# pynbody/topsy

Hardware: AMD Instinct MI355X
Metric: particles/sec splatted to 1024^2 buffer (higher is better)
Workload: dtype f32

## Files before the change

### include/topsy_splat.h

```cpp
#ifndef TOPSY_SPLAT_H
#define TOPSY_SPLAT_H

#include <stdint.h>

#ifdef __cplusplus
extern "C" {
#endif

typedef struct tsp_context tsp_context;

enum {
    TSP_OK = 0,
    TSP_EINVAL = -1,
    TSP_EHIP = -2,
    TSP_ENODEV = -3,
    TSP_ESTATE = -4,
    TSP_ECOMM = -5,
    TSP_ENOMEM = -6
};

enum {
    TSP_MODE_WEIGHTED = 0,
    TSP_MODE_DEPTH = 1,
    TSP_MODE_RGB = 2
// ... 120 lines not shown
int tsp_content_sort(tsp_context *ctx, int kind, float scale, int64_t *n_finite, int64_t *n_nonpositive);
int tsp_content_values(tsp_context *ctx, const int64_t *ranks, int n_ranks, float *out);

typedef struct {
    int64_t n_particles;
    int64_t n_small;
    int64_t n_mid;
    int64_t n_huge;
    int64_t n_culled;
    int64_t n_fragments;
    double ms_stream, ms_mid, ms_huge, ms_total;
    double ms_mega;
    int64_t n_mega;
    int64_t n_fragments_stream, n_fragments_mid, n_fragments_huge, n_fragments_mega;
    int64_t n_chunk_culled;
} tsp_stats;
int tsp_get_stats(tsp_context *ctx, tsp_stats *out);
int tsp_set_option(tsp_context *ctx, const char *name, int64_t value);

int tsp_measure_read_bandwidth(tsp_context *ctx, int64_t bytes, int iters, double *gbps_out);

#define TSP_UNIQUE_ID_BYTES 128
int tsp_comm_unique_id(char *id_out);
int tsp_comm_init(tsp_context *ctx, int n_ranks, int rank, const char *id);
int tsp_comm_reduce_image(tsp_context *ctx, int root, double *gpu_ms_out);
int tsp_comm_destroy(tsp_context *ctx);
int tsp_set_reduced_image(tsp_context *ctx, const float *sum);

typedef struct tsp_group tsp_group;
int tsp_group_create(int n_devices, const int *device_ids, int resolution, int n_channels, tsp_group **out);
// ... 26 lines not shown
```

### topsy_amd/_native.py

```python
import ctypes
import os

import numpy as np

_HERE = os.path.dirname(os.path.abspath(__file__))
LIB_PATH = os.environ.get("TOPSY_SPLAT_LIB") or os.path.join(_HERE, "libtopsy_splat.so")

MODE_WEIGHTED, MODE_DEPTH, MODE_RGB = 0, 1, 2
PIPE_DEFAULT, PIPE_GENERIC = 0, 1
SAMPLE_BILINEAR_MIP0, SAMPLE_BILINEAR_MIP = 0x10, 0x20
UNIQUE_ID_BYTES = 128
ABI_VERSION = 109
PRESENT_SCALAR, PRESENT_BIVARIATE, PRESENT_RGB, PRESENT_RGB_HDR = 0, 1, 2, 3
LAYER_QUAD, LAYER_LINES = 0, 1


class SurfaceParams(ctypes.Structure):
    _fields_ = [("smoothing_scale", ctypes.c_double), ("depth_scale", ctypes.c_float),
                ("light_direction", ctypes.c_float * 3), ("light_color", ctypes.c_float * 3), ("ambient_color", ctypes.c_float * 3),
                ("vmin", ctypes.c_float), ("vmax", ctypes.c_float), ("weighted_average", ctypes.c_int), ("log_scale", ctypes.c_int),
                ("lut_rgba", ctypes.POINTER(ctypes.c_float)), ("n_lut", ctypes.c_int)]


class PresentBase(ctypes.Structure):
    _fields_ = [("map", ctypes.c_int), ("vmin", ctypes.c_float), ("vmax", ctypes.c_float), ("density_vmin", ctypes.c_float),
                ("density_vmax", ctypes.c_float), ("gamma", ctypes.c_float), ("log_scale", ctypes.c_int), ("weighted", ctypes.c_int),
                ("lut_rgba", ctypes.POINTER(ctypes.c_float)), ("n_lut", ctypes.c_int)]
# ... 10 lines not shown

class BackendUnavailable(RuntimeError):
    """libtopsy_splat.so could not be loaded, or no MI355X-class GPU is visible."""


class BackendError(RuntimeError):
    """A C-ABI call returned a negative status."""


class Stats(ctypes.Structure):
    _fields_ = [("n_particles", ctypes.c_int64), ("n_small", ctypes.c_int64), ("n_mid", ctypes.c_int64),
                ("n_huge", ctypes.c_int64), ("n_culled", ctypes.c_int64), ("n_fragments", ctypes.c_int64),
                ("ms_stream", ctypes.c_double), ("ms_mid", ctypes.c_double), ("ms_huge", ctypes.c_double),
                ("ms_total", ctypes.c_double), ("ms_mega", ctypes.c_double), ("n_mega", ctypes.c_int64),
                ("n_fragments_stream", ctypes.c_int64), ("n_fragments_mid", ctypes.c_int64),
                ("n_fragments_huge", ctypes.c_int64), ("n_fragments_mega", ctypes.c_int64), ("n_chunk_culled", ctypes.c_int64)]

    def as_dict(self):
        return {k: getattr(self, k) for k, _ in self._fields_}


_fp = ctypes.POINTER(ctypes.c_float)
_i64p = ctypes.POINTER(ctypes.c_int64)
_u8p = ctypes.POINTER(ctypes.c_uint8)
_ctx = ctypes.c_void_p

SIGNATURES = {
    "tsp_last_error": (ctypes.c_char_p, []),
    "tsp_version": (ctypes.c_int, []),
    "tsp_stats_size": (ctypes.c_int, []),
    "tsp_device_count": (ctypes.c_int, []),
# ... 632 lines not shown
```

### topsy_amd/csrc/tsp_api.hip

```cpp
#include <stdarg.h>
#include <string.h>

#include <algorithm>
#include <cmath>
#include <vector>

#include "tsp_internal.h"

namespace tsp {

static thread_local char g_err[1024] = "";

void set_error(const char *fmt, ...) {
    va_list ap;
    va_start(ap, fmt);
    vsnprintf(g_err, sizeof(g_err), fmt, ap);
    va_end(ap);
}

int ensure_array(float **p, int64_t n) {
    if (*p) {
        TSP_HIP(hipFree(*p));
        *p = nullptr;
    }
// ... 123 lines not shown
    p.n = 0;
    ctx->ws.bounds_valid = false;
    ctx->surface_keys = false;
    ctx->strata_offsets.clear();
    ctx->cell_offsets.clear();
    ctx->cell_bits = 0;
}

}

using namespace tsp;

extern "C" {

const char *tsp_last_error(void) { return g_err; }
int tsp_version(void) { return 109; }
int tsp_stats_size(void) { return (int)sizeof(tsp_stats); }

int tsp_device_count(void) {
    int n = 0;
    if (hipGetDeviceCount(&n) != hipSuccess) {
        set_error("hipGetDeviceCount failed");
        return TSP_ENODEV;
    }
    return n;
}

static int create_resources(tsp_context *ctx, int device_id, int resolution, int n_channels) {
    hipDeviceProp_t prop;
    TSP_HIP(hipGetDeviceProperties(&prop, device_id));
    ctx->cu_count = prop.multiProcessorCount > 0 ? prop.multiProcessorCount : 256;
// ... 313 lines not shown

    Camera cam;
    for (int i = 0; i < 12; ++i) cam.m[i] = M[i];
    cam.sf = scale_factor;
    cam.R = ctx->R;
    cam.Rf = (float)ctx->R;
    cam.halfR = 0.5f * cam.Rf;

    TSP_HIP(hipEventRecord(ctx->ev[0], ctx->stream));
    if (clear)
        TSP_HIP(hipMemsetAsync(ctx->image64, 0, (size_t)ctx->R * ctx->R * ctx->C * sizeof(double), ctx->stream));
    TSP_HIP(hipMemsetAsync(ctx->counters, 0, sizeof(Counters), ctx->stream));
    ctx->stats = tsp_stats{};
    ctx->stats.n_particles = total;
    ctx->chunk_culled_particles = 0;
    int rc = TSP_OK;
    if (total > 0) {
        const int rule = (flags & TSP_SAMPLE_BILINEAR_MIP0) ? 1 : ((flags & TSP_SAMPLE_BILINEAR_MIP) ? 2 : 0);
        if ((flags & TSP_PIPE_GENERIC) || rule != 0) {
            std::vector<int64_t> pack(3 * (size_t)nr + 1);
            int64_t acc = 0;
            for (int i = 0; i < nr; ++i) {
                pack[i] = s[i];
                pack[nr + i] = l[i];
                pack[2 * nr + i] = acc;
                acc += l[i];
            }
            pack[3 * nr] = acc;
            if (ctx->ws.range_capacity < (int64_t)pack.size()) {
                const int64_t cap = (int64_t)pack.size() * 2 + 64;
// ... 11 lines not shown
    }
    if (rc) return rc;
    if ((rc = launch_image_convert(ctx, true))) return rc;
    ctx->image_is_reduced = false;
    TSP_HIP(hipEventRecord(ctx->ev[1], ctx->stream));
    TSP_HIP(hipStreamSynchronize(ctx->stream));
    float ms = 0.f;
    TSP_HIP(hipEventElapsedTime(&ms, ctx->ev[0], ctx->ev[1]));
    ctx->stats.ms_total = ms;
    Counters hc;
    TSP_HIP(hipMemcpy(&hc, ctx->counters, sizeof(hc), hipMemcpyDeviceToHost));
    ctx->stats.n_small = (int64_t)hc.n_small;
    ctx->stats.n_mid = (int64_t)hc.n_mid;
    ctx->stats.n_huge = (int64_t)hc.n_huge;
    ctx->stats.n_mega = 0;
    ctx->stats.n_culled = (int64_t)hc.n_culled + ctx->chunk_culled_particles;
    ctx->stats.n_chunk_culled = ctx->chunk_culled_particles;
    ctx->stats.n_fragments = (int64_t)hc.n_fragments;
    ctx->stats.n_fragments_stream = (int64_t)hc.n_frag_class[0];
    ctx->stats.n_fragments_mid = (int64_t)hc.n_frag_class[1];
    ctx->stats.n_fragments_huge = (int64_t)hc.n_frag_class[2];
    ctx->stats.n_fragments_mega = (int64_t)hc.n_frag_class[3];
    if (gpu_ms_out) *gpu_ms_out = ms;
    return TSP_OK;
}

int tsp_read_image(tsp_context *ctx, float *out) {
    TSP_REQUIRE(ctx && out, TSP_EINVAL, "NULL argument");
    TSP_HIP(hipSetDevice(ctx->device));
    TSP_HIP(hipMemcpy(out, ctx->image, (size_t)ctx->R * ctx->R * ctx->C * sizeof(float), hipMemcpyDeviceToHost));
    return TSP_OK;
}
// ... 361 lines not shown
    }
    if (!strcmp(name, "h2_walk")) {
        TSP_REQUIRE(value == 0 || value == 1, TSP_EINVAL, "%s out of range", name);
        ctx->h2_walk = (int)value;
        return TSP_OK;
    }
    if (!strcmp(name, "reorder_interleave")) {
        TSP_REQUIRE(value >= 0 && value <= 2, TSP_EINVAL, "%s out of range", name);
        ctx->reorder_interleave = (int)value;
        return TSP_OK;
    }
    if (!strcmp(name, "chunk_cull")) {
        ctx->chunk_cull = value != 0;
        return TSP_OK;
    }
    if (!strcmp(name, "overlap_mid_huge")) {
        ctx->overlap_mid_huge = value != 0;
        return TSP_OK;
    }
    if (!strcmp(name, "use_quantity")) {
        ctx->use_quantity = value != 0;
        return TSP_OK;
    }
    if (!strcmp(name, "active_channels")) {
        TSP_REQUIRE((value == 2 || value == 4) && value <= ctx->Ccap, TSP_EINVAL, "bad channel count %lld", (long long)value);
        ctx->C = (int)value;
        return TSP_OK;
    }
    set_error("unknown option '%s'", name);
    return TSP_EINVAL;
// ... 10 lines not shown
```

### topsy_amd/csrc/tsp_group.hip

```cpp
#include <algorithm>
#include <string>
#include <thread>
#include <vector>

#include "tsp_internal.h"

struct tsp_group {
    std::vector<tsp_context *> ctx;
    std::vector<int64_t> bounds;
    bool rccl = false;
    bool needs_reduce = false;
    int R = 0, Ccap = 0;
};

namespace {

using tsp::set_error;

template <typename F> int for_each_context(tsp_group *grp, F fn) {
    const int G = (int)grp->ctx.size();
    std::vector<int> rc(G, TSP_OK);
    std::vector<std::string> msg(G);
    std::vector<std::thread> th;
    th.reserve(G);
// ... 215 lines not shown
        return tsp_upload_band_magnitudes(grp->ctx[g], n_bands, cut.data(), weights);
    });
}

int tsp_group_get_stats(tsp_group *grp, tsp_stats *out) {
    TSP_REQUIRE(grp && out, TSP_EINVAL, "NULL argument");
    tsp_stats t = {};
    for (tsp_context *c : grp->ctx) {
        tsp_stats s;
        const int rc = tsp_get_stats(c, &s);
        if (rc) return rc;
        t.n_particles += s.n_particles; t.n_small += s.n_small; t.n_mid += s.n_mid; t.n_huge += s.n_huge; t.n_culled += s.n_culled;
        t.n_fragments += s.n_fragments; t.n_mega += s.n_mega;
        t.n_fragments_stream += s.n_fragments_stream; t.n_fragments_mid += s.n_fragments_mid;
        t.n_fragments_huge += s.n_fragments_huge; t.n_fragments_mega += s.n_fragments_mega; t.n_chunk_culled += s.n_chunk_culled;
        t.ms_stream = std::max(t.ms_stream, s.ms_stream); t.ms_mid = std::max(t.ms_mid, s.ms_mid);
        t.ms_huge = std::max(t.ms_huge, s.ms_huge); t.ms_mega = std::max(t.ms_mega, s.ms_mega);
        t.ms_total = std::max(t.ms_total, s.ms_total);
    }
    *out = t;
    return TSP_OK;
}

}
```

### topsy_amd/csrc/tsp_internal.h

```cpp
#pragma once
#include <hip/hip_runtime.h>
#include <stdint.h>

#include <initializer_list>
#include <vector>
#include <stdio.h>
#include <string>

#include "../../include/topsy_splat.h"
#include "tsp_math.h"

namespace tsp {

void set_error(const char *fmt, ...);

#define TSP_HIP(call)                                                                          \
    do {                                                                                       \
        hipError_t e_ = (call);                                                                \
        if (e_ != hipSuccess) {                                                                \
            tsp::set_error("%s failed: %s (%s:%d)", #call, hipGetErrorString(e_), __FILE__, __LINE__); \
            return TSP_EHIP;                                                                   \
        }                                                                                      \
    } while (0)

// ... 16 lines not shown
    bool wm_valid = false, wrgb_valid = false;
};

constexpr int BOUNDS_BLOCK = 512;

struct Record {
    float pcx, pcy, P, w0, w1;
};
struct Record4 {
    float pcx, pcy, P, w0, w1, w2;
};

struct Counters {
    unsigned long long n_small, n_mid, n_huge, n_culled, n_fragments, huge_count, next_chunk, mid_odd_weights;
    unsigned long long n_frag_class[4];
};

struct Workspace {
    void *mid_geom = nullptr, *mid_w = nullptr;
    int64_t mid_capacity = 0;
    void *huge_geom = nullptr, *huge_w = nullptr;
    int64_t huge_capacity = 0;
    void *hband_geom = nullptr, *hband_w = nullptr;
    int *hband_count = nullptr;
    int64_t hband_stride = 0; int hband_bands = 0;
    void *mband_geom = nullptr, *mband_w = nullptr;
    int *mband_count = nullptr;
    long long *mband_base = nullptr;
    int64_t mband_capacity = 0;
    int mtile_capacity = 0;
// ... 54 lines not shown
    bool count_fragments = false;
    float p_small = 16.0f;
    int64_t huge_band_budget = 6ll << 30;
    int huge_variant = 1;
    int h2_walk = 1;
    int huge_split = 0;
    int reorder_interleave = 2;
    int stream_blocks_per_cu = 0;
    int debug_gather_full_lut = 0;
    double mid_item_scale = 0.35;
    float mid_narrow_px = 64.0f;
    int mid_item_records = 0;
    int stream_batch_chunks = 8;
    bool chunk_cull = true;
    int64_t chunk_culled_particles = 0;
    bool overlap_mid_huge = false;
    int64_t slice_records = 0;
    int debug_fail_stage = 0;
    int64_t debug_fail_alloc = 0;
    int stream_occ[3][2] = {};
    bool debug_no_raster = false;
    int cu_count = 256;
    void *comm = nullptr;
    int n_ranks = 1, rank = 0;
    bool image_is_reduced = false;
};

namespace tsp {
struct DeviceScratch {
    void *p = nullptr;
// ... 62 lines not shown
```

### topsy_amd/csrc/tsp_pipeline.hip

```cpp
#include <string.h>

#include <algorithm>
#include <type_traits>
#include <vector>

#include "tsp_pipeline.h"

namespace tsp {

template <int CTRL, int ROW_MASK> __device__ __forceinline__ int dpp_or(int identity, int v) {
    return __builtin_amdgcn_update_dpp(identity, v, CTRL, ROW_MASK, 0xf, false);
}
template <typename Op> __device__ __forceinline__ int wave_scan_bits(int v, int identity, Op op) {
    v = op(v, dpp_or<0x111, 0xf>(identity, v));
    v = op(v, dpp_or<0x112, 0xf>(identity, v));
    v = op(v, dpp_or<0x114, 0xf>(identity, v));
    v = op(v, dpp_or<0x118, 0xf>(identity, v));
    v = op(v, dpp_or<0x142, 0xa>(identity, v));
    v = op(v, dpp_or<0x143, 0xc>(identity, v));
    return v;
}
__device__ __forceinline__ float wave_min(float v) {
    const int r = wave_scan_bits(__float_as_int(v), __float_as_int(__builtin_inff()),
                                 [](int a, int b) { return __float_as_int(fminf(__int_as_float(a), __int_as_float(b))); });
// ... 45 lines not shown
    int count_frag;
    int emit_small;
    const int *alive;
    const unsigned long long *cull_info;
};

static_assert(CHUNK == BOUNDS_BLOCK, "block bounds are kept per chunk-sized block");
constexpr int T23_FLOATS = 17 * 17 + 9 * 9;

struct CullArgs {
    const int64_t *ranges; int n_ranges; int n_chunks;
    Camera cam;
    const float4 *bounds; int64_t n_particles;
    int *alive; unsigned long long *info;
    int *wg_count;
};

__device__ __forceinline__ bool box_outside_view(const Camera &c, float4 lo, float4 hi) {
    if (!(c.sf > 0.0f)) return false;
    const float bx = 0.5f * lo.x + 0.5f * hi.x, by = 0.5f * lo.y + 0.5f * hi.y, bz = 0.5f * lo.z + 0.5f * hi.z;
    const float ex = 0.5f * hi.x - 0.5f * lo.x, ey = 0.5f * hi.y - 0.5f * lo.y, ez = 0.5f * hi.z - 0.5f * lo.z;
    const float s = (c.sf * lo.w) * 2.0f;
    const float px = 4.0f / c.Rf;
    bool out = false;
#pragma unroll
    for (int row = 0; row < 3; ++row) {
        const float a = c.m[4 * row] * bx, b = c.m[4 * row + 1] * by, d = c.m[4 * row + 2] * bz, t = c.m[4 * row + 3];
        const float centre = ((a + b) + d) + t;
        const float ext = (__builtin_fabsf(c.m[4 * row]) * ex + __builtin_fabsf(c.m[4 * row + 1]) * ey) + __builtin_fabsf(c.m[4 * row + 2]) * ez;
        const float mag = (((__builtin_fabsf(a) + __builtin_fabsf(b)) + __builtin_fabsf(d)) + __builtin_fabsf(t)) + ext;
        if (row < 2) {
            const float reach = (ext + s) + (1e-4f * (mag + s) + px);
            out = out || (centre - reach > 1.0f) || (centre + reach < -1.0f);
        } else {
            const float reach = ext + (1e-4f * mag + 1e-6f);
            out = out || (centre - reach > 1.0f) || (centre + reach < 0.0f);
        }
    }
    return out;
}

__device__ __forceinline__ bool chunk_alive(const CullArgs &a, int c, int &cnt) {
    const int n_ranges = a.n_ranges;
    const int64_t *starts = a.ranges, *lens = starts + n_ranges, *cprefix = starts + 2 * n_ranges;
    int lo = 0, hi = n_ranges - 1;
    while (lo < hi) {
        const int mid = (lo + hi + 1) >> 1;
        if (cprefix[mid] <= c) lo = mid; else hi = mid - 1;
    }
    const int64_t in_range = (int64_t)(c - cprefix[lo]) * CHUNK;
    const int64_t first = starts[lo] + in_range;
    cnt = (int)min((int64_t)CHUNK, lens[lo] - in_range);
    const int64_t b0 = first / BOUNDS_BLOCK, b1 = (first + cnt - 1) / BOUNDS_BLOCK;
    float4 blo = a.bounds[2 * b0], bhi = a.bounds[2 * b0 + 1];
    if (b1 != b0) {
        const float4 l1 = a.bounds[2 * b1], h1 = a.bounds[2 * b1 + 1];
        blo = make_float4(fminf(blo.x, l1.x), fminf(blo.y, l1.y), fminf(blo.z, l1.z), fmaxf(blo.w, l1.w));
        bhi = make_float4(fmaxf(bhi.x, h1.x), fmaxf(bhi.y, h1.y), fmaxf(bhi.z, h1.z), 0.0f);
    }
    return !box_outside_view(a.cam, blo, bhi);
}

template <int PASS>
__global__ __launch_bounds__(256) void chunk_cull_kernel(CullArgs a) {
    __shared__ int s_cnt[4];
    const int c = blockIdx.x * 256 + threadIdx.x, lane = threadIdx.x & 63, wv = threadIdx.x >> 6;
    int cnt = 0;
    const bool alive = (c < a.n_chunks) && chunk_alive(a, c, cnt);
    const unsigned long long m = __ballot(alive);
    if (lane == 0) s_cnt[wv] = __popcll(m);
    if (PASS == 0) {
        unsigned long long dropped = alive ? 0ull : (unsigned long long)cnt;
        for (int o = 32; o; o >>= 1) dropped += __shfl_xor((long long)dropped, o);
        if (lane == 0 && dropped) atomicAdd(&a.info[1], dropped);
    }
    __syncthreads();
    if (PASS == 0) {
        if (threadIdx.x == 0) a.wg_count[blockIdx.x] = s_cnt[0] + s_cnt[1] + s_cnt[2] + s_cnt[3];
    } else if (alive) {
        int pos = a.wg_count[blockIdx.x] + __popcll(m & ((1ull << lane) - 1ull));
        for (int w = 0; w < wv; ++w) pos += s_cnt[w];
        a.alive[pos] = c;
    }
}

__global__ __launch_bounds__(1024) void chunk_cull_scan_kernel(int *wg_count, int n, unsigned long long *info) {
    __shared__ int s_wave[16];
    __shared__ int s_carry;
    const int tid = threadIdx.x, lane = tid & 63, wv = tid >> 6;
    if (tid == 0) s_carry = 0;
    __syncthreads();
    for (int base = 0; base < n; base += 1024) {
        const int i = base + tid;
        const int v = i < n ? wg_count[i] : 0;
        int incl = v;
        for (int o = 1; o < 64; o <<= 1) {
            const int t = __shfl_up(incl, o);
            if (lane >= o) incl += t;
        }
        if (lane == 63) s_wave[wv] = incl;
        __syncthreads();
        int before = s_carry;
        for (int w = 0; w < wv; ++w) before += s_wave[w];
        if (i < n) wg_count[i] = before + incl - v;
        __syncthreads();
        if (tid == 1023) s_carry = before + incl;
        __syncthreads();
    }
    if (tid == 0) info[0] = (unsigned long long)s_carry;
}

template <int MODE, int WC>
__global__ __launch_bounds__(SBLOCK, TSP_S_OCC) void splat_stream_kernel(StreamArgs ) {
    typedef const __attribute__((address_space(4))) StreamArgs CArgs;
    auto KA = []() -> CArgs * {
        CArgs *p = (CArgs *)__builtin_amdgcn_kernarg_segment_ptr();
        asm volatile("" : "+s"(p));
        return p;
    };
    constexpr int C = (MODE == TSP_MODE_RGB) ? 4 : 2;
    constexpr int NW = (MODE == TSP_MODE_RGB) ? 2 : 1;
    constexpr int WIN = WinSize<WC>::value;
    extern __shared__ __attribute__((aligned(16))) double smem_d[];
    double *win = smem_d;
// ... 373 lines not shown
        n_small += __shfl_xor((long long)n_small, o);
        n_cull += __shfl_xor((long long)n_cull, o);
        n_frag += __shfl_xor((long long)n_frag, o);
    }
    if (lane == 0) {
        Counters *cntp = KA()->cnt;
        if (n_small) atomicAdd(&cntp->n_small, n_small);
        if (n_cull) atomicAdd(&cntp->n_culled, n_cull);
        if (n_frag) { atomicAdd(&cntp->n_fragments, n_frag); atomicAdd(&cntp->n_frag_class[0], n_frag); }
#ifdef TSP_S_DEBUG
        if (dbg_slots) atomicAdd(&cntp->n_frag_class[1], dbg_slots);
#endif
    }
}

__global__ __launch_bounds__(256) void rect_count_corners_kernel(const float4 *__restrict__ geom, long long n, int R, int *__restrict__ D) {
    const long long i = (long long)blockIdx.x * 256 + threadIdx.x;
    if (i >= n) return;
    const float4 g = geom[i];
    const float half = 0.5f * __builtin_fabsf(g.z);
    int ilo, ihi, jlo, jhi;
    cover_range(g.x, half, R, ilo, ihi);
    cover_range(g.y, half, R, jlo, jhi);
    if (ilo > ihi || jlo > jhi) return;
    const int S = R + 1;
    atomicAdd(&D[jlo * S + ilo], 1);
    atomicAdd(&D[jlo * S + ihi + 1], -1);
    atomicAdd(&D[(jhi + 1) * S + ilo], -1);
    atomicAdd(&D[(jhi + 1) * S + ihi + 1], 1);
}
// ... 76 lines not shown
        pack[2 * n_ranges + i] = n_chunks64;
        n_chunks64 += (h_lens[i] + CHUNK - 1) / CHUNK;
    }
    pack[3 * n_ranges] = n_chunks64;
    TSP_REQUIRE(n_chunks64 < (1ll << 30), TSP_EINVAL, "too many chunks");
    const int n_chunks = (int)n_chunks64;
    int rc;
    if ((rc = check_workspace(ctx))) return rc;
    if (ws.range_capacity < (int64_t)pack.size()) {
        const int64_t cap = (int64_t)pack.size() * 2 + 64;
        if ((rc = alloc_group(ctx, {{"range_prefix", (void **)&ws.range_prefix, (size_t)cap * sizeof(int64_t)}}, {{&ws.range_capacity, cap}}))) return rc;
    }
    TSP_HIP(hipMemcpyAsync(ws.range_prefix, pack.data(), pack.size() * sizeof(int64_t), hipMemcpyHostToDevice, st));
    if (ws.chunk_capacity < n_chunks) {
        const int64_t cap = (int64_t)n_chunks + n_chunks / 4 + 64;
        if ((rc = alloc_group(ctx, {{"alive_list", (void **)&ws.alive_list, (size_t)(cap + cap / 256 + 2) * sizeof(int)}}, {{&ws.chunk_capacity, cap}})))
            return rc;
    }
    if ((rc = ensure_weights(ctx, MODE == TSP_MODE_RGB))) return rc;
    if (ws.mid_capacity == 0 && (rc = alloc_list(ctx, &ws.mid_geom, &ws.mid_w, &ws.mid_capacity, std::max<int64_t>(total / 4, 1 << 16),
                                                 SITE("mid_geom"), SITE("mid_w"))))
        return rc;
    if (ws.huge_capacity == 0 && (rc = alloc_list(ctx, &ws.huge_geom, &ws.huge_w, &ws.huge_capacity, std::max<int64_t>(total / 16, 1 << 16),
                                                  SITE("huge_geom"), SITE("huge_w"))))
        return rc;

    Particles parts = ctx->p;
    if (!ctx->use_quantity) parts.q = nullptr;
    const bool second_channel = (MODE == TSP_MODE_DEPTH) || (MODE == TSP_MODE_RGB) || (ctx->p.q != nullptr && ctx->use_quantity);
    const int WCr = (MODE == TSP_MODE_RGB) ? 4 : (second_channel ? 2 : 1);
    const int WIN = (WCr == 1) ? WinSize<1>::value : WinSize<C>::value;
    const size_t smem_s = (size_t)WCr * WIN * WIN * sizeof(double) + T23_FLOATS * sizeof(float);
    if (!(ctx->kernel_attr_done & (1u << MODE))) {
        TSP_HIP(hipFuncSetAttribute((const void *)splat_stream_kernel<MODE, C>, hipFuncAttributeMaxDynamicSharedMemorySize, (int)((size_t)C * WinSize<C>::value * WinSize<C>::value * sizeof(double) + T23_FLOATS * sizeof(float))));
        TSP_HIP(hipFuncSetAttribute((const void *)splat_stream_kernel<MODE, 1>, hipFuncAttributeMaxDynamicSharedMemorySize, (int)((size_t)WinSize<1>::value * WinSize<1>::value * sizeof(double) + T23_FLOATS * sizeof(float))));
        ctx->kernel_attr_done |= 1u << MODE;
    }

    const bool cull = ctx->chunk_cull && n_chunks >= 4096;
    unsigned long long cull_info_h[2] = {0, 0};
    ctx->chunk_culled_particles = 0;
    TSP_HIP(hipEventRecord(ctx->ev[7], st));
    if (cull) {
        if ((rc = ensure_block_bounds(ctx))) return rc;
        if (!ws.cull_info && (rc = alloc_group(ctx, {{"cull_info", (void **)&ws.cull_info, 2 * sizeof(unsigned long long)}}, {}))) return rc;
        TSP_HIP(hipMemsetAsync(ws.cull_info, 0, 2 * sizeof(unsigned long long), st));
        CullArgs ca;
        ca.ranges = ws.range_prefix; ca.n_ranges = n_ranges; ca.n_chunks = n_chunks; ca.cam = cam;
        ca.bounds = ws.block_bounds; ca.n_particles = ctx->p.n; ca.alive = ws.alive_list; ca.info = ws.cull_info;
        ca.wg_count = ws.alive_list + ws.chunk_capacity;
        const int n_wg = (n_chunks + 255) / 256;
        hipLaunchKernelGGL(chunk_cull_kernel<0>, dim3(n_wg), dim3(256), 0, st, ca);
        hipLaunchKernelGGL(chunk_cull_scan_kernel, dim3(1), dim3(1024), 0, st, ca.wg_count, n_wg, ws.cull_info);
        hipLaunchKernelGGL(chunk_cull_kernel<1>, dim3(n_wg), dim3(256), 0, st, ca);
        TSP_HIP(hipGetLastError());
    }

    Counters hc, carry;
    memset(&carry, 0, sizeof(carry));
    for (int attempt = 0; attempt < 2; ++attempt) {
        StreamArgs sa;
        sa.p = parts;
        sa.alive = cull ? ws.alive_list : nullptr; sa.cull_info = ws.cull_info;
        sa.ranges = ws.range_prefix; sa.n_ranges = n_ranges; sa.n_chunks = n_chunks;
        const int min_cpb = std::max(1, std::min(8, n_chunks / (ctx->cu_count * 2)));
        int per_cu = ctx->stream_blocks_per_cu;
        if (per_cu <= 0) {
            int &occ = ctx->stream_occ[MODE][WCr == 1 ? 0 : 1];
// ... 5 lines not shown
        }
        const int resident = ctx->cu_count * per_cu;
        sa.dynamic = (min_cpb >= 8 && n_chunks > resident * 8) ? 1 : 0;
        sa.chunks_per_block = sa.dynamic ? std::max(4, ctx->stream_batch_chunks) : min_cpb;
        const int grid_s = sa.dynamic ? resident : (n_chunks + sa.chunks_per_block - 1) / sa.chunks_per_block;
        sa.cam = cam; sa.mips = ctx->mips; sa.img = ctx->image64;
        sa.mid_geom = (float4 *)ws.mid_geom; sa.mid_w = (float *)ws.mid_w; sa.mid_capacity = ws.mid_capacity;
        sa.huge_geom = (float4 *)ws.huge_geom; sa.huge_w = (float *)ws.huge_w; sa.huge_capacity = ws.huge_capacity;
        sa.cnt = ctx->counters; sa.p_small = ctx->p_small;
        sa.count_frag = ctx->count_fragments ? 1 : 0;
        sa.emit_small = (attempt == 0 && !ctx->debug_no_raster) ? 1 : 0;
        TSP_HIP(hipEventRecord(ctx->ev[2], st));
        if (WCr == 1) hipLaunchKernelGGL((splat_stream_kernel<MODE, 1>), dim3(grid_s), dim3(SBLOCK), smem_s, st, sa);
        else hipLaunchKernelGGL((splat_stream_kernel<MODE, C>), dim3(grid_s), dim3(SBLOCK), smem_s, st, sa);
        TSP_HIP(hipGetLastError());
        TSP_HIP(hipEventRecord(ctx->ev[3], st));
        TSP_HIP(hipMemcpyAsync(&hc, ctx->counters, sizeof(hc), hipMemcpyDeviceToHost, st));
        if (cull && attempt == 0) TSP_HIP(hipMemcpyAsync(cull_info_h, ws.cull_info, sizeof(cull_info_h), hipMemcpyDeviceToHost, st));
        TSP_HIP(hipStreamSynchronize(st));
        ctx->chunk_culled_particles = (int64_t)cull_info_h[1];
        const bool mid_over = (int64_t)hc.n_mid > ws.mid_capacity, huge_over = (int64_t)hc.n_huge > ws.huge_capacity;
        if (!mid_over && !huge_over) break;
        TSP_REQUIRE(attempt == 0, TSP_ENOMEM, "record lists overflowed twice");
        if (mid_over && (rc = alloc_list(ctx, &ws.mid_geom, &ws.mid_w, &ws.mid_capacity, (int64_t)hc.n_mid + (int64_t)hc.n_mid / 8 + 1024,
                                         SITE("mid_geom_replay"), SITE("mid_w_replay"))))
            return rc;
        if (huge_over && (rc = alloc_list(ctx, &ws.huge_geom, &ws.huge_w, &ws.huge_capacity, (int64_t)hc.n_huge + (int64_t)hc.n_huge / 8 + 1024,
                                          SITE("huge_geom_replay"), SITE("huge_w_replay"))))
            return rc;
        TSP_HIP(hipMemsetAsync(ctx->counters, 0, sizeof(Counters), st));
        carry = hc;
    }

    if (carry.n_small || carry.n_fragments) {
        hc.n_small += carry.n_small;
        hc.n_fragments += carry.n_fragments;
        hc.n_frag_class[0] += carry.n_frag_class[0];
        TSP_HIP(hipMemcpyAsync(ctx->counters, &hc, sizeof(hc), hipMemcpyHostToDevice, st));
        TSP_HIP(hipStreamSynchronize(st));
    }
    TileArgs ta;
    ta.cam = cam; ta.mips = ctx->mips; ta.img = ctx->image64; ta.cnt = ctx->counters; ta.tiles_x = 0; ta.split = 1;
    ta.count_frag = ctx->count_fragments ? 1 : 0;
    ta.hband_count = nullptr; ta.hband_stride = 0; ta.hband_base = nullptr; ta.n_tiles = 0; ta.item_tile = nullptr; ta.item_base = nullptr;
    ta.disc_k2 = (ctx->lut_zero_outside_disc && !ctx->count_fragments) ? 0.5235f * 0.5235f : 0.0f;
    hipStream_t st_mid = ctx->overlap_mid_huge ? ctx->stream2 : st;
    if (ctx->overlap_mid_huge) {
        TSP_HIP(hipEventRecord(ctx->ev[8], st));
        TSP_HIP(hipStreamWaitEvent(st_mid, ctx->ev[8], 0));
// ... 53 lines not shown
```

### topsy_amd/multigpu.py

```python
import math
from concurrent.futures import ThreadPoolExecutor

import numpy as np

from . import _native, distributed

_COUNT_KEYS = ("n_particles", "n_small", "n_mid", "n_huge", "n_culled", "n_fragments", "n_mega",
               "n_fragments_stream", "n_fragments_mid", "n_fragments_huge", "n_fragments_mega", "n_chunk_culled")


class MultiGpuContext:
    def __init__(self, resolution, n_channels, device_ids, assignment="contiguous", interleave_block=4096):
        device_ids = [int(d) for d in device_ids]
        if len(device_ids) < 2:
            raise ValueError("MultiGpuContext needs at least two contexts (use _native.Context for one GPU)")
        if assignment not in ("contiguous", "interleaved"):
            raise ValueError(f"unknown shard assignment '{assignment}'")
        self.assignment = assignment
        self.interleave_block = int(interleave_block)
        self._cyclic = False
        self._cyclic_ranges = False
        self._n_uploaded = 0
        self.device_ids = device_ids
        self.contexts = [_native.Context(resolution, n_channels, d) for d in device_ids]
# ... 236 lines not shown
```

Before: 20.73 billion.

## Route chunks of sub-pixel particles to a dedicated single-pixel point splat kernel

Extends the chunk-cull pass to classify visible chunks whose maximum projected particle size is at most one pixel and compacts them into a separate point list via a second prefix scan. A new wave-per-chunk-range point kernel draws these particles by sampling a single kernel texel per particle and merging same-pixel atomics within a wave. Register double-buffering of the next unit's loads hides memory latency. This skips the general stream kernel's per-particle classification and footprint logic for tiny particles, at the cost of extra cull-kernel work, a second kernel launch and assumptions about coverage of exactly one pixel.

After: 20.22 billion (median of 2 runs). 0.975x the previous value.

```diff
diff --git a/include/topsy_splat.h b/include/topsy_splat.h
--- a/include/topsy_splat.h
+++ b/include/topsy_splat.h
@@ -158,6 +158,7 @@
     int64_t n_mega;
     int64_t n_fragments_stream, n_fragments_mid, n_fragments_huge, n_fragments_mega;
     int64_t n_chunk_culled;
+    int64_t n_point_chunks, n_point_particles;
 } tsp_stats;
 int tsp_get_stats(tsp_context *ctx, tsp_stats *out);
 int tsp_set_option(tsp_context *ctx, const char *name, int64_t value);
diff --git a/topsy_amd/_native.py b/topsy_amd/_native.py
--- a/topsy_amd/_native.py
+++ b/topsy_amd/_native.py
@@ -10,7 +10,7 @@
 PIPE_DEFAULT, PIPE_GENERIC = 0, 1
 SAMPLE_BILINEAR_MIP0, SAMPLE_BILINEAR_MIP = 0x10, 0x20
 UNIQUE_ID_BYTES = 128
-ABI_VERSION = 109
+ABI_VERSION = 110
 PRESENT_SCALAR, PRESENT_BIVARIATE, PRESENT_RGB, PRESENT_RGB_HDR = 0, 1, 2, 3
 LAYER_QUAD, LAYER_LINES = 0, 1
 
@@ -51,7 +51,8 @@
                 ("ms_stream", ctypes.c_double), ("ms_mid", ctypes.c_double), ("ms_huge", ctypes.c_double),
                 ("ms_total", ctypes.c_double), ("ms_mega", ctypes.c_double), ("n_mega", ctypes.c_int64),
                 ("n_fragments_stream", ctypes.c_int64), ("n_fragments_mid", ctypes.c_int64),
-                ("n_fragments_huge", ctypes.c_int64), ("n_fragments_mega", ctypes.c_int64), ("n_chunk_culled", ctypes.c_int64)]
+                ("n_fragments_huge", ctypes.c_int64), ("n_fragments_mega", ctypes.c_int64), ("n_chunk_culled", ctypes.c_int64),
+                ("n_point_chunks", ctypes.c_int64), ("n_point_particles", ctypes.c_int64)]
 
     def as_dict(self):
         return {k: getattr(self, k) for k, _ in self._fields_}
diff --git a/topsy_amd/csrc/tsp_api.hip b/topsy_amd/csrc/tsp_api.hip
--- a/topsy_amd/csrc/tsp_api.hip
+++ b/topsy_amd/csrc/tsp_api.hip
@@ -161,7 +161,7 @@
 extern "C" {
 
 const char *tsp_last_error(void) { return g_err; }
-int tsp_version(void) { return 109; }
+int tsp_version(void) { return 110; }
 int tsp_stats_size(void) { return (int)sizeof(tsp_stats); }
 
 int tsp_device_count(void) {
@@ -505,6 +505,7 @@
     ctx->stats = tsp_stats{};
     ctx->stats.n_particles = total;
     ctx->chunk_culled_particles = 0;
+    ctx->point_chunks_drawn = ctx->point_particles = 0;
     int rc = TSP_OK;
     if (total > 0) {
         const int rule = (flags & TSP_SAMPLE_BILINEAR_MIP0) ? 1 : ((flags & TSP_SAMPLE_BILINEAR_MIP) ? 2 : 0);
@@ -546,8 +547,10 @@
     ctx->stats.n_mid = (int64_t)hc.n_mid;
     ctx->stats.n_huge = (int64_t)hc.n_huge;
     ctx->stats.n_mega = 0;
-    ctx->stats.n_culled = (int64_t)hc.n_culled + ctx->chunk_culled_particles;
+    ctx->stats.n_culled = (int64_t)hc.n_culled + (int64_t)hc.n_point_culled + ctx->chunk_culled_particles;
     ctx->stats.n_chunk_culled = ctx->chunk_culled_particles;
+    ctx->stats.n_point_chunks = ctx->point_chunks_drawn;
+    ctx->stats.n_point_particles = ctx->point_particles;
     ctx->stats.n_fragments = (int64_t)hc.n_fragments;
     ctx->stats.n_fragments_stream = (int64_t)hc.n_frag_class[0];
     ctx->stats.n_fragments_mid = (int64_t)hc.n_frag_class[1];
@@ -939,6 +942,10 @@
         ctx->chunk_cull = value != 0;
         return TSP_OK;
     }
+    if (!strcmp(name, "point_chunks")) {
+        ctx->point_chunks = value != 0;
+        return TSP_OK;
+    }
     if (!strcmp(name, "overlap_mid_huge")) {
         ctx->overlap_mid_huge = value != 0;
         return TSP_OK;
diff --git a/topsy_amd/csrc/tsp_group.hip b/topsy_amd/csrc/tsp_group.hip
--- a/topsy_amd/csrc/tsp_group.hip
+++ b/topsy_amd/csrc/tsp_group.hip
@@ -253,6 +253,7 @@
         t.n_fragments += s.n_fragments; t.n_mega += s.n_mega;
         t.n_fragments_stream += s.n_fragments_stream; t.n_fragments_mid += s.n_fragments_mid;
         t.n_fragments_huge += s.n_fragments_huge; t.n_fragments_mega += s.n_fragments_mega; t.n_chunk_culled += s.n_chunk_culled;
+        t.n_point_chunks += s.n_point_chunks; t.n_point_particles += s.n_point_particles;
         t.ms_stream = std::max(t.ms_stream, s.ms_stream); t.ms_mid = std::max(t.ms_mid, s.ms_mid);
         t.ms_huge = std::max(t.ms_huge, s.ms_huge); t.ms_mega = std::max(t.ms_mega, s.ms_mega);
         t.ms_total = std::max(t.ms_total, s.ms_total);
diff --git a/topsy_amd/csrc/tsp_internal.h b/topsy_amd/csrc/tsp_internal.h
--- a/topsy_amd/csrc/tsp_internal.h
+++ b/topsy_amd/csrc/tsp_internal.h
@@ -54,6 +54,7 @@
 struct Counters {
     unsigned long long n_small, n_mid, n_huge, n_culled, n_fragments, huge_count, next_chunk, mid_odd_weights;
     unsigned long long n_frag_class[4];
+    unsigned long long n_point_culled;
 };
 
 struct Workspace {
@@ -138,6 +139,9 @@
     int stream_batch_chunks = 8;
     bool chunk_cull = true;
     int64_t chunk_culled_particles = 0;
+    bool point_chunks = true;
+    int64_t point_chunks_drawn = 0, point_particles = 0;
+    int point_occ[2] = {};
     bool overlap_mid_huge = false;
     int64_t slice_records = 0;
     int debug_fail_stage = 0;
diff --git a/topsy_amd/csrc/tsp_pipeline.hip b/topsy_amd/csrc/tsp_pipeline.hip
--- a/topsy_amd/csrc/tsp_pipeline.hip
+++ b/topsy_amd/csrc/tsp_pipeline.hip
@@ -83,6 +83,9 @@
     const float4 *bounds; int64_t n_particles;
     int *alive; unsigned long long *info;
     int *wg_count;
+    int *point; int *wg_count_point;
+    int do_cull;
+    int classify;
 };
 
 __device__ __forceinline__ bool box_outside_view(const Camera &c, float4 lo, float4 hi) {
@@ -109,7 +112,7 @@
     return out;
 }
 
-__device__ __forceinline__ bool chunk_alive(const CullArgs &a, int c, int &cnt) {
+__device__ __forceinline__ int chunk_class(const CullArgs &a, int c, int &cnt) {
     const int n_ranges = a.n_ranges;
     const int64_t *starts = a.ranges, *lens = starts + n_ranges, *cprefix = starts + 2 * n_ranges;
     int lo = 0, hi = n_ranges - 1;
@@ -127,56 +130,68 @@
         blo = make_float4(fminf(blo.x, l1.x), fminf(blo.y, l1.y), fminf(blo.z, l1.z), fmaxf(blo.w, l1.w));
         bhi = make_float4(fmaxf(bhi.x, h1.x), fmaxf(bhi.y, h1.y), fmaxf(bhi.z, h1.z), 0.0f);
     }
-    return !box_outside_view(a.cam, blo, bhi);
+    if (a.do_cull && box_outside_view(a.cam, blo, bhi)) return 0;
+    const float p_max = ((a.cam.sf * blo.w) * 2.0f) * a.cam.Rf;
+    return (a.classify && a.cam.sf > 0.0f && __builtin_fabsf(p_max) <= 1.0f) ? 2 : 1;
 }
 
 template <int PASS>
 __global__ __launch_bounds__(256) void chunk_cull_kernel(CullArgs a) {
-    __shared__ int s_cnt[4];
+    __shared__ int s_cnt[4], s_cnt_point[4];
     const int c = blockIdx.x * 256 + threadIdx.x, lane = threadIdx.x & 63, wv = threadIdx.x >> 6;
     int cnt = 0;
-    const bool alive = (c < a.n_chunks) && chunk_alive(a, c, cnt);
-    const unsigned long long m = __ballot(alive);
-    if (lane == 0) s_cnt[wv] = __popcll(m);
+    const int cls = (c < a.n_chunks) ? chunk_class(a, c, cnt) : 0;
+    const bool alive = cls == 1, point = cls == 2;
+    const unsigned long long m = __ballot(alive), mp = __ballot(point);
+    if (lane == 0) { s_cnt[wv] = __popcll(m); s_cnt_point[wv] = __popcll(mp); }
     if (PASS == 0) {
-        unsigned long long dropped = alive ? 0ull : (unsigned long long)cnt;
-        for (int o = 32; o; o >>= 1) dropped += __shfl_xor((long long)dropped, o);
+        unsigned long long dropped = cls ? 0ull : (unsigned long long)cnt, in_point = point ? (unsigned long long)cnt : 0ull;
+        for (int o = 32; o; o >>= 1) { dropped += __shfl_xor((long long)dropped, o); in_point += __shfl_xor((long long)in_point, o); }
         if (lane == 0 && dropped) atomicAdd(&a.info[1], dropped);
+        if (lane == 0 && in_point) atomicAdd(&a.info[3], in_point);
     }
     __syncthreads();
     if (PASS == 0) {
-        if (threadIdx.x == 0) a.wg_count[blockIdx.x] = s_cnt[0] + s_cnt[1] + s_cnt[2] + s_cnt[3];
-    } else if (alive) {
-        int pos = a.wg_count[blockIdx.x] + __popcll(m & ((1ull << lane) - 1ull));
-        for (int w = 0; w < wv; ++w) pos += s_cnt[w];
-        a.alive[pos] = c;
-    }
-}
-
-__global__ __launch_bounds__(1024) void chunk_cull_scan_kernel(int *wg_count, int n, unsigned long long *info) {
+        if (threadIdx.x == 0) {
+            a.wg_count[blockIdx.x] = s_cnt[0] + s_cnt[1] + s_cnt[2] + s_cnt[3];
+            a.wg_count_point[blockIdx.x] = s_cnt_point[0] + s_cnt_point[1] + s_cnt_point[2] + s_cnt_point[3];
+        }
+    } else if (cls) {
+        const int *wg = point ? a.wg_count_point : a.wg_count, *sc = point ? s_cnt_point : s_cnt;
+        int pos = wg[blockIdx.x] + __popcll((point ? mp : m) & ((1ull << lane) - 1ull));
+        for (int w = 0; w < wv; ++w) pos += sc[w];
+        (point ? a.point : a.alive)[pos] = c;
+    }
+}
+
+__global__ __launch_bounds__(1024) void chunk_cull_scan_kernel(int *wg_count_general, int *wg_count_point, int n, unsigned long long *info) {
     __shared__ int s_wave[16];
     __shared__ int s_carry;
     const int tid = threadIdx.x, lane = tid & 63, wv = tid >> 6;
-    if (tid == 0) s_carry = 0;
-    __syncthreads();
-    for (int base = 0; base < n; base += 1024) {
-        const int i = base + tid;
-        const int v = i < n ? wg_count[i] : 0;
-        int incl = v;
-        for (int o = 1; o < 64; o <<= 1) {
-            const int t = __shfl_up(incl, o);
-            if (lane >= o) incl += t;
-        }
-        if (lane == 63) s_wave[wv] = incl;
+    for (int list = 0; list < 2; ++list) {
+        int *wg_count = list ? wg_count_point : wg_count_general;
+        if (tid == 0) s_carry = 0;
         __syncthreads();
-        int before = s_carry;
-        for (int w = 0; w < wv; ++w) before += s_wave[w];
-        if (i < n) wg_count[i] = before + incl - v;
+        for (int base = 0; base < n; base += 1024) {
+            const int i = base + tid;
+            const int v = i < n ? wg_count[i] : 0;
+            int incl = v;
+            for (int o = 1; o < 64; o <<= 1) {
+                const int t = __shfl_up(incl, o);
+                if (lane >= o) incl += t;
+            }
+            if (lane == 63) s_wave[wv] = incl;
+            __syncthreads();
+            int before = s_carry;
+            for (int w = 0; w < wv; ++w) before += s_wave[w];
+            if (i < n) wg_count[i] = before + incl - v;
+            __syncthreads();
+            if (tid == 1023) s_carry = before + incl;
+            __syncthreads();
+        }
+        if (tid == 0) info[2 * list] = (unsigned long long)s_carry;
         __syncthreads();
-        if (tid == 1023) s_carry = before + incl;
-        __syncthreads();
-    }
-    if (tid == 0) info[0] = (unsigned long long)s_carry;
+    }
 }
 
 template <int MODE, int WC>
@@ -580,6 +595,132 @@
     }
 }
 
+struct PointArgs {
+    Particles p;
+    const int64_t *ranges; int n_ranges;
+    Camera cam;
+    const float *mips;
+    double *img;
+    Counters *cnt;
+    int count_frag;
+    const int *list;
+    const unsigned long long *cull_info;
+};
+constexpr int POINT_STEPS = 4;
+static_assert(CHUNK % (64 * POINT_STEPS) == 0, "a chunk is a whole number of units");
+
+template <int MODE, int WC>
+__global__ __launch_bounds__(256) void splat_point_kernel(PointArgs a) {
+    static_assert(MODE == TSP_MODE_WEIGHTED && (WC == 1 || WC == 2), "the point path draws the weighted mode only");
+    constexpr int C = 2, UNIT = 64 * POINT_STEPS, UNITS = CHUNK / UNIT, NATTR = 4 + WC;
+    const int lane = threadIdx.x & 63;
+    const long long n_list = (long long)a.cull_info[2];
+    const long long n_waves = (long long)gridDim.x * (blockDim.x >> 6), wave = (long long)blockIdx.x * (blockDim.x >> 6) + (threadIdx.x >> 6);
+    const int c_begin = (int)(n_list * wave / n_waves), c_end = (int)(n_list * (wave + 1) / n_waves);
+    if (c_begin >= c_end) return;
+    const float t3 = a.mips[5376 + lane];
+    const int R = a.cam.R;
+    const float Rf = a.cam.Rf;
+
+    auto locate = [&](int c, int64_t &first, int &cnt) {
+        const int n_ranges = a.n_ranges;
+        const int64_t *starts = a.ranges, *lens = starts + n_ranges, *cprefix = starts + 2 * n_ranges;
+        int lo = 0, hi = n_ranges - 1;
+        while (lo < hi) {
+            const int mid = (lo + hi + 1) >> 1;
+            if (cprefix[mid] <= c) lo = mid; else hi = mid - 1;
+        }
+        const int64_t in_range = (int64_t)(c - cprefix[lo]) * CHUNK;
+        first = starts[lo] + in_range;
+        cnt = (int)min((int64_t)CHUNK, lens[lo] - in_range);
+    };
+    float L[POINT_STEPS][NATTR];
+    auto load_unit = [&](int64_t first, int cnt, int u) {
+#pragma unroll
+        for (int s = 0; s < POINT_STEPS; ++s) {
+            const int64_t i = first + min(u * UNIT + s * 64 + lane, cnt - 1);
+            L[s][0] = a.p.x[i]; L[s][1] = a.p.y[i]; L[s][2] = a.p.z[i]; L[s][3] = a.p.h[i];
+            L[s][4] = a.p.wm[i];
+            if (WC == 2) L[s][NATTR - 1] = a.p.q[i];
+        }
+    };
+
+    unsigned long long n_small = 0, n_cull = 0;
+    int64_t first, first_next = 0;
+    int cnt, cnt_next = 0;
+    locate(a.list[c_begin], first, cnt);
+    load_unit(first, cnt, 0);
+    for (int c = c_begin, u = 0;;) {
+        float A[POINT_STEPS][NATTR];
+#pragma unroll
+        for (int s = 0; s < POINT_STEPS; ++s)
+#pragma unroll
+            for (int k = 0; k < NATTR; ++k) A[s][k] = L[s][k];
+        const int base = u * UNIT, cnt_now = cnt;
+        bool more = true;
+        if (u + 1 < UNITS && (u + 1) * UNIT < cnt) { ++u; load_unit(first, cnt, u); }
+        else if (c + 1 < c_end) {
+            ++c; u = 0;
+            locate(a.list[c], first_next, cnt_next);
+            first = first_next; cnt = cnt_next;
+            load_unit(first, cnt, 0);
+        } else more = false;
+
+#pragma unroll
+        for (int s = 0; s < POINT_STEPS; ++s) {
+            const bool in_chunk = base + s * 64 + lane < cnt_now;
+            const Proj pr = project<false>(a.cam, A[s][0], A[s][1], A[s][2], A[s][3]);
+            const float fi = __builtin_floorf(pr.pcx), fj = __builtin_floorf(pr.pcy);
+            const bool hit = in_chunk && pr.keep && fi >= 0.0f && fi < Rf && fj >= 0.0f && fj < Rf &&
+                             covers(pr.pcx, pr.half, fi) && covers(pr.pcy, pr.half, fj);
+            n_small += hit ? 1ull : 0ull;
+            n_cull += (in_chunk && !hit) ? 1ull : 0ull;
+            if (__ballot(hit) == 0ull) continue;
+            const float ip = 1.0f / pr.P;
+            const float dx = (fi + 0.5f) - pr.pcx, dy = (fj + 0.5f) - pr.pcy;
+            const int tx = floor_clamp_s(((dx + pr.half) * ip) * 8.0f, 7), ty = floor_clamp_s(((dy + pr.half) * ip) * 8.0f, 7);
+            const float kv = __shfl(t3, hit ? ty * 8 + tx : 0);
+            const float val = kv * A[s][4];
+            const float val1 = (WC == 2) ? val * A[s][NATTR - 1] : 0.0f;
+            const bool on = hit && ((WC == 1) ? (val != 0.0f) : (kv != 0.0f));
+            const int key = hit ? (int)fj * R + (int)fi : -1;
+            unsigned long long todo = __ballot(on);
+            for (int round = 0; round < 4 && todo != 0ull; ++round) {
+                const int src = __ffsll((long long)todo) - 1;
+                const int k0 = __builtin_amdgcn_readlane(key, src);
+                const bool match = on && key == k0;
+                const unsigned long long mm = __ballot(match);
+                todo &= ~mm;
+                float sum = val, sum1 = val1;
+                if (__popcll(mm) != 1) {
+                    sum = wave_sum(match ? val : 0.0f);
+                    if (WC == 2) sum1 = wave_sum(match ? val1 : 0.0f);
+                }
+                if (lane == src) {
+                    gatomic_add(a.img + (size_t)key * C, (double)sum);
+                    if (WC == 2) gatomic_add(a.img + (size_t)key * C + 1, (double)sum1);
+                }
+            }
+            if ((todo >> lane) & 1ull) {
+                gatomic_add(a.img + (size_t)key * C, (double)val);
+                if (WC == 2) gatomic_add(a.img + (size_t)key * C + 1, (double)val1);
+            }
+        }
+        if (!more) break;
+    }
+    for (int o = 32; o; o >>= 1) {
+        n_small += __shfl_xor((long long)n_small, o);
+        n_cull += __shfl_xor((long long)n_cull, o);
+    }
+    if (lane == 0) {
+        if (n_small) {
+            atomicAdd(&a.cnt->n_small, n_small);
+            if (a.count_frag) { atomicAdd(&a.cnt->n_fragments, n_small); atomicAdd(&a.cnt->n_frag_class[0], n_small); }
+        }
+        if (n_cull) atomicAdd(&a.cnt->n_point_culled, n_cull);
+    }
+}
+
 __global__ __launch_bounds__(256) void rect_count_corners_kernel(const float4 *__restrict__ geom, long long n, int R, int *__restrict__ D) {
     const long long i = (long long)blockIdx.x * 256 + threadIdx.x;
     if (i >= n) return;
@@ -686,7 +827,7 @@
     TSP_HIP(hipMemcpyAsync(ws.range_prefix, pack.data(), pack.size() * sizeof(int64_t), hipMemcpyHostToDevice, st));
     if (ws.chunk_capacity < n_chunks) {
         const int64_t cap = (int64_t)n_chunks + n_chunks / 4 + 64;
-        if ((rc = alloc_group(ctx, {{"alive_list", (void **)&ws.alive_list, (size_t)(cap + cap / 256 + 2) * sizeof(int)}}, {{&ws.chunk_capacity, cap}})))
+        if ((rc = alloc_group(ctx, {{"alive_list", (void **)&ws.alive_list, (size_t)(2 * (cap + cap / 256 + 2)) * sizeof(int)}}, {{&ws.chunk_capacity, cap}})))
             return rc;
     }
     if ((rc = ensure_weights(ctx, MODE == TSP_MODE_RGB))) return rc;
@@ -709,21 +850,28 @@
         ctx->kernel_attr_done |= 1u << MODE;
     }
 
-    const bool cull = ctx->chunk_cull && n_chunks >= 4096;
-    unsigned long long cull_info_h[2] = {0, 0};
+    const bool passes = n_chunks >= 4096;
+    const bool point_path = passes && ctx->point_chunks && MODE == TSP_MODE_WEIGHTED && ctx->p_small > 1.0f && !ctx->debug_no_raster;
+    const bool cull = passes && (ctx->chunk_cull || point_path);
+    unsigned long long cull_info_h[4] = {0, 0, 0, 0};
     ctx->chunk_culled_particles = 0;
+    ctx->point_chunks_drawn = ctx->point_particles = 0;
     TSP_HIP(hipEventRecord(ctx->ev[7], st));
+    const int *point_list = nullptr;
     if (cull) {
         if ((rc = ensure_block_bounds(ctx))) return rc;
-        if (!ws.cull_info && (rc = alloc_group(ctx, {{"cull_info", (void **)&ws.cull_info, 2 * sizeof(unsigned long long)}}, {}))) return rc;
-        TSP_HIP(hipMemsetAsync(ws.cull_info, 0, 2 * sizeof(unsigned long long), st));
+        if (!ws.cull_info && (rc = alloc_group(ctx, {{"cull_info", (void **)&ws.cull_info, 4 * sizeof(unsigned long long)}}, {}))) return rc;
+        TSP_HIP(hipMemsetAsync(ws.cull_info, 0, 4 * sizeof(unsigned long long), st));
         CullArgs ca;
         ca.ranges = ws.range_prefix; ca.n_ranges = n_ranges; ca.n_chunks = n_chunks; ca.cam = cam;
         ca.bounds = ws.block_bounds; ca.n_particles = ctx->p.n; ca.alive = ws.alive_list; ca.info = ws.cull_info;
         ca.wg_count = ws.alive_list + ws.chunk_capacity;
+        ca.point = ca.wg_count + ws.chunk_capacity / 256 + 2; ca.wg_count_point = ca.point + ws.chunk_capacity;
+        ca.do_cull = ctx->chunk_cull ? 1 : 0; ca.classify = point_path ? 1 : 0;
+        point_list = ca.point;
         const int n_wg = (n_chunks + 255) / 256;
         hipLaunchKernelGGL(chunk_cull_kernel<0>, dim3(n_wg), dim3(256), 0, st, ca);
-        hipLaunchKernelGGL(chunk_cull_scan_kernel, dim3(1), dim3(1024), 0, st, ca.wg_count, n_wg, ws.cull_info);
+        hipLaunchKernelGGL(chunk_cull_scan_kernel, dim3(1), dim3(1024), 0, st, ca.wg_count, ca.wg_count_point, n_wg, ws.cull_info);
         hipLaunchKernelGGL(chunk_cull_kernel<1>, dim3(n_wg), dim3(256), 0, st, ca);
         TSP_HIP(hipGetLastError());
     }
@@ -759,11 +907,24 @@
         if (WCr == 1) hipLaunchKernelGGL((splat_stream_kernel<MODE, 1>), dim3(grid_s), dim3(SBLOCK), smem_s, st, sa);
         else hipLaunchKernelGGL((splat_stream_kernel<MODE, C>), dim3(grid_s), dim3(SBLOCK), smem_s, st, sa);
         TSP_HIP(hipGetLastError());
+        if (point_path && attempt == 0) {
+            PointArgs pa;
+            pa.p = parts; pa.ranges = ws.range_prefix; pa.n_ranges = n_ranges; pa.cam = cam; pa.mips = ctx->mips; pa.img = ctx->image64;
+            pa.cnt = ctx->counters; pa.count_frag = sa.count_frag; pa.list = point_list; pa.cull_info = ws.cull_info;
+            int &occ = ctx->point_occ[WCr == 1 ? 0 : 1];
+            const void *fn = (WCr == 1) ? (const void *)splat_point_kernel<TSP_MODE_WEIGHTED, 1> : (const void *)splat_point_kernel<TSP_MODE_WEIGHTED, 2>;
+            if (occ <= 0 && (hipOccupancyMaxActiveBlocksPerMultiprocessor(&occ, fn, 256, 0) != hipSuccess || occ <= 0)) { (void)hipGetLastError(); occ = 4; }
+            const int grid_p = std::max(1, std::min(ctx->cu_count * occ, (n_chunks + 3) / 4));
+            if (WCr == 1) hipLaunchKernelGGL((splat_point_kernel<TSP_MODE_WEIGHTED, 1>), dim3(grid_p), dim3(256), 0, st, pa);
+            else hipLaunchKernelGGL((splat_point_kernel<TSP_MODE_WEIGHTED, 2>), dim3(grid_p), dim3(256), 0, st, pa);
+            TSP_HIP(hipGetLastError());
+        }
         TSP_HIP(hipEventRecord(ctx->ev[3], st));
         TSP_HIP(hipMemcpyAsync(&hc, ctx->counters, sizeof(hc), hipMemcpyDeviceToHost, st));
         if (cull && attempt == 0) TSP_HIP(hipMemcpyAsync(cull_info_h, ws.cull_info, sizeof(cull_info_h), hipMemcpyDeviceToHost, st));
         TSP_HIP(hipStreamSynchronize(st));
         ctx->chunk_culled_particles = (int64_t)cull_info_h[1];
+        ctx->point_chunks_drawn = (int64_t)cull_info_h[2]; ctx->point_particles = (int64_t)cull_info_h[3];
         const bool mid_over = (int64_t)hc.n_mid > ws.mid_capacity, huge_over = (int64_t)hc.n_huge > ws.huge_capacity;
         if (!mid_over && !huge_over) break;
         TSP_REQUIRE(attempt == 0, TSP_ENOMEM, "record lists overflowed twice");
@@ -777,7 +938,8 @@
         carry = hc;
     }
 
-    if (carry.n_small || carry.n_fragments) {
+    if (carry.n_small || carry.n_fragments || carry.n_point_culled) {
+        hc.n_point_culled += carry.n_point_culled;
         hc.n_small += carry.n_small;
         hc.n_fragments += carry.n_fragments;
         hc.n_frag_class[0] += carry.n_frag_class[0];
diff --git a/topsy_amd/multigpu.py b/topsy_amd/multigpu.py
--- a/topsy_amd/multigpu.py
+++ b/topsy_amd/multigpu.py
@@ -6,7 +6,8 @@
 from . import _native, distributed
 
 _COUNT_KEYS = ("n_particles", "n_small", "n_mid", "n_huge", "n_culled", "n_fragments", "n_mega",
-               "n_fragments_stream", "n_fragments_mid", "n_fragments_huge", "n_fragments_mega", "n_chunk_culled")
+               "n_fragments_stream", "n_fragments_mid", "n_fragments_huge", "n_fragments_mega", "n_chunk_culled",
+               "n_point_chunks", "n_point_particles")
 
 
 class MultiGpuContext:
```
